# Chthi/Ofighters

Measured on AMD Instinct MI355X. Metric: arena-steps/sec (env.step+obs+policy fwd) at 4096 arenas, 1/2/4/8 MI355X, higher is better.
Workload: dtype f32; 1 GPU; 4096 arenas x 8 ships per GPU, random-bot actions + step + 2D obs rasterise (u8 maps) + bi-head policy forward for 8 ship(s)/arena, trunk shared per arena (BASELINE configs[3]); arenas_per_gpu=4096, ships=8, laser_cap=512, episode_ticks=200, parallelism=arena-sharded x1, RCCL all-reduce of episodic scores only, laser_overflow=0, last_episode_score_sum=70993, last_episode_arenas=4096

## Files before the change

### include/ofx.h

```cpp
#ifndef OFX_H
#define OFX_H

#include <stddef.h>
#include <stdint.h>

#ifdef __cplusplus
extern "C" {
#endif

#define OFX_VERSION 1

enum {
  OFX_OK = 0,
  OFX_ERR_INVALID = -1,
  OFX_ERR_NO_DEVICE = -2,
  OFX_ERR_HIP = -3,
  OFX_ERR_STATE = -4,
  OFX_ERR_OVERFLOW = -5
};

typedef struct ofx_config {
  int32_t n_arenas;
  int32_t n_ships;
  int32_t laser_cap;
// ... 102 lines not shown
int ofx_field_desc(ofx_handle *h, int field, ofx_tensor_desc *out);
int ofx_map_desc(ofx_handle *h, int map_type, int which, ofx_tensor_desc *out);

int ofx_overflow_count(ofx_handle *h, int64_t *count_host);

int ofx_episode_scores(ofx_handle *h, int64_t *sums);
int ofx_scores_allreduce(ofx_handle *h, void *nccl_comm, int64_t *sums);

int ofx_scratch_feed(ofx_handle *h, const int32_t *layers_host, int32_t n_layers,
                     const double *weights, const double *biases, const double *x,
                     int32_t batch, double *y, int32_t *argmax);
int ofx_scratch_feed_obs(ofx_handle *h, const int32_t *layers_host, int32_t n_layers,
                         const double *weights, const double *biases, double *y,
                         int32_t *argmax);

typedef struct ofx_policy_desc {
  int32_t n_floats;
  int32_t offset[64];
  int32_t count[64];
  int32_t n_tensors;
} ofx_policy_desc;
int ofx_policy_layout(const ofx_handle *h, ofx_policy_desc *desc_host);
int ofx_policy_forward(ofx_handle *h, const float *weights, const uint8_t *ship_mask,
                       float *act_values, int32_t *iaction, int32_t *ipointer,
                       float *heatmap);
int ofx_policy_pin_weights(ofx_handle *h, const float *weights);
#define OFX_OPT_TRUNK_PLAIN 1
#define OFX_OPT_FRAMES_REF  2
#define OFX_OPT_TRUNK_FUSE  4
#define OFX_OPT_BILINEAR_LEGACY 3
#define OFX_OPT_POLICY_BF16 5
#define OFX_OPT_FIT_PLAIN 6
#define OFX_OPT_TRUNK_SPARSE 7
int ofx_policy_trunk_stats(ofx_handle *h, int64_t *counts_host);
int ofx_set_option(ofx_handle *h, int32_t option, int32_t value);
int ofx_policy_explore(ofx_handle *h, double epsilon, uint64_t seed, uint32_t tick, int32_t collecting,
                       const uint8_t *ship_mask, int32_t *iaction, int32_t *ipointer);
int ofx_policy_actions(ofx_handle *h, const int32_t *iaction, const int32_t *ipointer,
                       const uint8_t *ship_mask, ofx_action *actions);

typedef struct ofx_transition {
  int32_t tick_prev, tick_next;
  int32_t frame_prev, frame_next;
  int32_t ship;
  int32_t iaction, px, py;
  int32_t reward;
  int32_t done;
  float head_prev[8], head_next[8];
} ofx_transition;
int ofx_replay_create(ofx_handle *h, int32_t capacity, int32_t frames);
int ofx_replay_destroy(ofx_handle *h);
int ofx_replay_capture(ofx_handle *h, uint32_t tick, const uint8_t *ship_mask, const int32_t *iaction,
                       const int32_t *ipointer);
int ofx_agents_first_done(ofx_handle *h, const uint8_t *ship_mask, uint8_t *seen, int32_t *count_host);
int ofx_replay_count(ofx_handle *h, int32_t *count_host, int64_t *appended_host);
int ofx_replay_rows_host(ofx_handle *h, int32_t arena, ofx_transition *rows_host, int32_t *n_host);
int ofx_replay_frame_host(ofx_handle *h, int32_t arena, int32_t tick, void *ship_bits_host, void *laser_bits_host);
int ofx_replay_sample(ofx_handle *h, uint64_t seed, uint32_t draw, int32_t batch, int32_t *slot, int32_t *n_sampled);
int ofx_replay_gather(ofx_handle *h, const int32_t *slot, int32_t batch, ofx_transition *rows, void *bits_prev,
                      void *bits_next);
int ofx_replay_gather_valid(ofx_handle *h, const int32_t *slot, const int32_t *n_sampled, int32_t batch, int32_t first,
                            int32_t max_rows, ofx_transition *rows, void *bits_prev, void *bits_next,
                            int32_t *n_rows_host);

int ofx_replay_prioritize(ofx_handle *h, float alpha, float eps);
int ofx_replay_sample_prioritized(ofx_handle *h, uint64_t seed, uint32_t draw, int32_t batch, double beta, int32_t *slot,
// ... 41 lines not shown
```

### ofighters_amd/_native.py

```python
import ctypes as C
import os

_HERE = os.path.dirname(os.path.abspath(__file__))
LIB_PATH = os.path.join(_HERE, "libofx.so")

OFX_OK = 0
OFX_ERR_INVALID = -1
OFX_ERR_NO_DEVICE = -2
OFX_ERR_HIP = -3
OFX_ERR_STATE = -4
OFX_ERR_OVERFLOW = -5

BOT_IDLE, BOT_RANDOM, BOT_TURRET, BOT_RUNNER, BOT_THRUST, BOT_SHOOT = range(6)
BEHAVIOURS = {None: BOT_IDLE, "idle": BOT_IDLE, "random": BOT_RANDOM, "turret": BOT_TURRET,
              "runner": BOT_RUNNER, "thrust": BOT_THRUST, "shoot": BOT_SHOOT}

(F_SHIP_X, F_SHIP_Y, F_SHIP_PX, F_SHIP_PY, F_SHIP_ALIVE, F_REWARD, F_SCORE, F_N_LASERS, F_LASER_X, F_LASER_Y,
 F_LASER_OWNER, F_LASER_DEAD, F_KILLER, F_TIME, F_LAST_SCORES, F_HULL, F_LASER_DX, F_LASER_DY,
 F_OBS_REWARD) = range(19)

MAP_U8, MAP_F32, MAP_F64, MAP_BITS = range(4)
OPT_TRUNK_PLAIN, OPT_FRAMES_REF, OPT_BILINEAR_LEGACY, OPT_TRUNK_FUSE, OPT_POLICY_BF16, OPT_FIT_PLAIN, OPT_TRUNK_SPARSE = 1, 2, 3, 4, 5, 6, 7


class OfxError(Exception):
    def __init__(self, code, msg):
        super().__init__(msg)
        self.code = code


class OfxConfig(C.Structure):
    _fields_ = [(n, C.c_int32) for n in (
        "n_arenas", "n_ships", "laser_cap", "width", "height", "ship_radius", "laser_radius",
        "ship_speed", "laser_speed", "reward_death", "reward_kill", "reward_aim",
        "reward_trajectory", "episode_ticks", "device", "arena_base")]


class OfxAction(C.Structure):
    _fields_ = [("px", C.c_int32), ("py", C.c_int32), ("shoot", C.c_uint8), ("thrust", C.c_uint8),
                ("valid", C.c_uint8), ("_pad", C.c_uint8)]


class OfxTransition(C.Structure):
    _fields_ = [("tick_prev", C.c_int32), ("tick_next", C.c_int32), ("frame_prev", C.c_int32),
                ("frame_next", C.c_int32), ("ship", C.c_int32), ("iaction", C.c_int32),
                ("px", C.c_int32), ("py", C.c_int32), ("reward", C.c_int32), ("done", C.c_int32),
                ("head_prev", C.c_float * 8), ("head_next", C.c_float * 8)]


class OfxTensorDesc(C.Structure):
    _fields_ = [("data", C.c_void_p), ("dtype", C.c_int32), ("itemsize", C.c_int32), ("ndim", C.c_int32),
                ("device", C.c_int32), ("shape", C.c_int64 * 4), ("stride", C.c_int64 * 4)]


DT_U8, DT_I16, DT_I32, DT_I64, DT_F32, DT_F64 = range(6)
# ... 114 lines not shown
```

### ofighters_amd/csrc/ofx_head.h

```cpp
#pragma once
#include "ofx_internal.h"

struct HeadParams2 {
  int S;
  const float *up1;
  const float *w2mf, *b2;
  const float *w2raw;
  const float *w3mf, *b3;
  const float *w3raw;
  const float *w4eff_c, *b4;
  const float *w4raw;
  const float *w2fr, *w3fr;
  const float *efr;
  float *u2fr;
  float *vfr;
  float *c4;
  const uint8_t *mask;
  int32_t *live;
  int live_ready;
  unsigned long long *best;
  float *heat;
  const int32_t *probe;
  float *ptr_probe;
  int frames_ref;
  int legacy;
  int bf16;
  int event_base;
  int ablate;
  unsigned long long *dbg;
};

size_t ofx_head_frame_bytes(size_t S, size_t *u2fr, size_t *vfr, size_t *c4);
int ofx_head_compact(ofx_handle *h, int S, const uint8_t *mask, int32_t *live);
int ofx_launch_head(ofx_handle *h, const HeadParams2 &p);
```

### ofighters_amd/csrc/ofx_head.hip

```cpp
#include "ofx_head.h"
#include "ofx_lowp.h"
#include "ofx_diag.h"
#include <stdlib.h>


typedef float f32x4 __attribute__((ext_vector_type(4)));
typedef float f32x2 __attribute__((ext_vector_type(2)));
#define HD_PS 400
constexpr int HC4_ZERO = 800;
constexpr int HC4_COL = 816, HC4_CPITCH = 416;
constexpr int HC4_STRIDE = HC4_COL + 2 * HC4_CPITCH + 16;
__device__ __forceinline__ int hc4_at(int ln, int t) { return ln < 2 ? ln * 400 + t : HC4_COL + (ln - 2) * HC4_CPITCH + t; }
__device__ __forceinline__ int hc4_pad(int k) { return k < 16 ? HC4_ZERO + k : k < 32 ? HC4_COL + 400 + k - 16 : HC4_COL + HC4_CPITCH + 400 + k - 32; }

__device__ __forceinline__ void hc4_zero_block(const HeadParams2 &p, int tid, int threads) {
  if (blockIdx.x == 0)
    for (int e = tid; e < HC4_STRIDE; e += threads) p.c4[(size_t)p.S * HC4_STRIDE + e] = 0.f;
}

__device__ __forceinline__ float hd_max_raw(float x, float floor) {
  float pinf;
  asm("s_mov_b32 %0, 0x7f800000" : "=s"(pinf));
  return __builtin_amdgcn_fmed3f(x, floor, pinf);
}
// ... 205 lines not shown
}

constexpr int HG_THREADS = 256;
constexpr int HG_L1 = 0;
constexpr int HG_U3 = 0;
constexpr int HG_RB = 6400;
constexpr int HG_CB = HG_RB + 4 * 102 * 4;
constexpr int HG_TOTAL = HG_CB + 4 * 102 * 4;
static_assert(2 * 52 * 52 <= 6400, "l1p fits under u3l");

template <int CIN, int COUT, class G>
__device__ __forceinline__ float hg_corner(G get, int n, int yc, int xc, const float *w, float bias, int co, int legacy) {
  float acc = bias;
  for (int dy = 0; dy < 3; dy++) {
    const int uy = yc + dy - 1;
    if (uy < 0 || uy >= 2 * n) continue;
    int ya, yb; float wy;
    hf_taps(uy, n, ya, yb, wy, legacy);
    for (int dx = 0; dx < 3; dx++) {
      const int ux = xc + dx - 1;
      if (ux < 0 || ux >= 2 * n) continue;
      int xa, xb; float wx;
      hf_taps(ux, n, xa, xb, wx, legacy);
      for (int ci = 0; ci < CIN; ci++) {
        const float a = get(ya, xa, ci), b = get(ya, xb, ci), d = get(yb, xa, ci), g = get(yb, xb, ci);
        const float top = a + (b - a) * wx, bot = d + (g - d) * wx;
        acc += w[((dy * 3 + dx) * CIN + ci) * COUT + co] * (top + (bot - top) * wy);
      }
    }
  }
  return fmaxf(acc, 0.f);
}

__global__ __launch_bounds__(HG_THREADS) void k_head_frames(HeadParams2 p) {
  __shared__ __align__(16) float sm[HG_TOTAL];
  __shared__ float efr_s[192], w4s[72];
  const int s = hd_ship(p, (int)((blockIdx.x & ~7u) | ((blockIdx.x + (blockIdx.x >> 3)) & 7u)));
  const int tid = threadIdx.x, lane = tid & 63;
  hc4_zero_block(p, tid, HG_THREADS);
  if (s < 0) return;
  const int wv = __builtin_amdgcn_readfirstlane(tid >> 6);
  const int n16 = lane & 15, kq = lane >> 4;
  float *l1p = sm + HG_L1, *u2rb = sm + HG_RB, *u2cb = sm + HG_CB, *u3l = sm + HG_U3;

  {
    constexpr int NB = 6 * 52 + 46 * 6, NE = 2 * NB, PER = (NE + HG_THREADS - 1) / HG_THREADS;
    float v[PER];
    int at[PER];
#pragma unroll
    for (int u = 0; u < PER; u++) {
      const int e = min(u * HG_THREADS + tid, NE - 1);
      const int ci = e / NB, k = e - ci * NB;
      int r, c;
      if (k < 6 * 52) { const int rr = k / 52; r = rr < 3 ? rr : rr + 46; c = k - rr * 52; }
      else { const int k2 = k - 6 * 52, cc = k2 % 6; r = 3 + k2 / 6; c = cc < 3 ? cc : cc + 46; }
      at[u] = (ci * 52 + r) * 52 + c;
      v[u] = p.up1[(size_t)s * 5000 + (ci * 50 + min(max(r - 1, 0), 49)) * 50 + min(max(c - 1, 0), 49)];
    }
#pragma unroll
    for (int u = 0; u < PER; u++)
      if (u * HG_THREADS + tid < NE) l1p[at[u]] = v[u];
  }
  if (tid < 192) efr_s[tid] = p.efr[tid];
  if (tid < 72) w4s[tid] = p.w4raw[tid];
  __syncthreads();

  float bw2[5];
#pragma unroll
  for (int jj = 0; jj < 5; jj++) bw2[jj] = p.w2fr[(wv * 20 + 4 * jj + kq) * 16 + n16];
  float bw3[9];
#pragma unroll
  for (int jj = 0; jj < 9; jj++) bw3[jj] = p.w3fr[(wv * 36 + 4 * jj + kq) * 16 + n16];
#pragma unroll 1
  for (int m = 0; m < 4; m++) {
    const int v = wv;
    const int pp = min(16 * m + n16, 49);
    const int i = v == 0 ? 0 : v == 1 ? 49 : pp, j = v == 2 ? 0 : v == 3 ? 49 : pp;
    const float bias = p.b2[n16 & 3];
    f32x4 d = {bias, bias, bias, bias};
#pragma unroll
    for (int jj = 0; jj < 5; jj++) {
      const int tap = min(2 * jj + (kq >> 1), 8);
      const float a = l1p[((kq & 1) * 52 + i + tap / 3) * 52 + j + tap % 3];
      d = __builtin_amdgcn_mfma_f32_16x16x4f32(a, bw2[jj], d, 0, 0, 0);
    }
    const int co = n16 & 3, pa = n16 >> 3, pb = (n16 >> 2) & 1;
#pragma unroll
    for (int r = 0; r < 4; r++) {
      const int q = 16 * m + 4 * kq + r;
      if (q >= 50) continue;
      const float val = fmaxf(d[r], 0.f);
      if (v < 2) {
        u2rb[((2 * v + pa) * 102 + 2 * q + pb + 1) * 4 + co] = val;
      } else {
        u2cb[((2 * (v - 2) + pb) * 102 + 2 * q + pa + 1) * 4 + co] = val;
      }
    }
  }
  __syncthreads();
  if (tid < 64) {
    const int co = tid & 3, cx = (tid >> 2) & 1, cy = (tid >> 3) & 1, bx = (tid >> 4) & 1, by = tid >> 5;
    const int y = by ? 98 + cy : cy, x = bx ? 98 + cx : cx;
    const int rb = by ? 2 + cy : cy, cb = bx ? 2 + cx : cx;
    const bool fy = y == 0 || y == 99, fx = x == 0 || x == 99;
    float val;
    if (fy && fx) {
      auto get = [&](int yy, int xx, int ci) { return l1p[(ci * 52 + yy + 1) * 52 + xx + 1]; };
      val = hg_corner<2, 4>(get, 50, y, x, p.w2raw, p.b2[co], co, p.legacy);
    } else if (fx) {
      val = u2cb[(cb * 102 + y + 1) * 4 + co];
    } else {
      val = u2rb[(rb * 102 + x + 1) * 4 + co];
    }
    if (fy && fx) { u2rb[(rb * 102 + x + 1) * 4 + co] = val; u2cb[(cb * 102 + y + 1) * 4 + co] = val; }
    else if (fx) u2rb[(rb * 102 + x + 1) * 4 + co] = val;
    else u2cb[(cb * 102 + y + 1) * 4 + co] = val;
  }
  __syncthreads();
  if (tid < 128) {
    const int co = tid & 3, b = (tid >> 2) & 3, hi = (tid >> 4) & 1, isc = tid >> 5;
    if (isc < 2) {
      float *ln = (isc ? u2cb : u2rb) + b * 102 * 4;
      ln[(hi ? 101 : 0) * 4 + co] = ln[(hi ? 100 : 1) * 4 + co];
    }
  }
  for (int e = tid; e < 4 * 100 * 4; e += HG_THREADS) {
    const int ln = e / 400, r = e - ln * 400;
    const float *src = ln < 2 ? u2rb + (ln ? 3 : 0) * 408 : u2cb + (ln == 3 ? 3 : 0) * 408;
    p.u2fr[(size_t)s * 1600 + e] = src[4 + r];
  }
  __syncthreads();

#pragma unroll 1
  for (int m = 0; m < 7; m++) {
    const int v = wv;
    const int qq = min(16 * m + n16, 99);
    const float *band = (v < 2 ? u2rb : u2cb);
    const int b0 = (v & 1) ? 2 : 0;
    const float bias = p.b3[n16 & 7];
    f32x4 d = {bias, bias, bias, bias};
#pragma unroll
    for (int jj = 0; jj < 9; jj++) {
      const int ty = jj / 3, tx = jj % 3;
      const int tf = v < 2 ? ty : tx, ta = v < 2 ? tx : ty;
      const int bsel = (v & 1) ? b0 + min(tf, 1) : b0 + max(tf - 1, 0);
      const float a = band[(bsel * 102 + qq + ta) * 4 + kq];
      d = __builtin_amdgcn_mfma_f32_16x16x4f32(a, bw3[jj], d, 0, 0, 0);
    }
    const int co = n16 & 7, par = n16 >> 3;
#pragma unroll
    for (int r = 0; r < 4; r++) {
      const int q = 16 * m + 4 * kq + r;
      if (q < 100) u3l[(v * 200 + 2 * q + par) * 8 + co] = fmaxf(d[r], 0.f);
    }
  }
  __syncthreads();
  if (tid < 32) {
    const int co = tid & 7, c = tid >> 3;
    const int y = (c & 1) ? 199 : 0, x = (c & 2) ? 199 : 0;
    auto get = [&](int yy, int xx, int ci) {
      return u2rb[((yy < 50 ? yy : yy - 96) * 102 + xx + 1) * 4 + ci];
    };
    const float val = hg_corner<4, 8>(get, 100, y, x, p.w3raw, p.b3[co], co, p.legacy);
    u3l[(((c & 1) ? 1 : 0) * 200 + x) * 8 + co] = val;
    u3l[(((c & 2) ? 3 : 2) * 200 + y) * 8 + co] = val;
  }
  __syncthreads();
  if (tid < 252) {
    const int tp = tid % 9, c0 = tid / 9;
    float wt[8];
#pragma unroll
    for (int ci = 0; ci < 8; ci++) wt[ci] = w4s[tp * 8 + ci];
    float *dst = p.vfr + (size_t)s * 7200 + tid;
    for (int cell = c0; cell < 4 * 200; cell += 28) {
      const f32x4 ua = *reinterpret_cast<const f32x4 *>(u3l + cell * 8), ub = *reinterpret_cast<const f32x4 *>(u3l + cell * 8 + 4);
      float acc = 0.f;
#pragma unroll
      for (int ci = 0; ci < 4; ci++) acc = fmaf(wt[ci], ua[ci], acc);
#pragma unroll
      for (int ci = 0; ci < 4; ci++) acc = fmaf(wt[4 + ci], ub[ci], acc);
      dst[(cell - c0) * 9] = acc;
    }
  }

  for (int e = tid; e < 4 * 400; e += HG_THREADS) {
    const int ln = e / 400, t = e - ln * 400, isc = ln >> 1, side = ln & 1, jq = t >> 1, b = t & 1;
    float acc = 0.f;
    if (!isc || (t > 0 && t < 399)) {
      const float *E = efr_s + ((isc * 2 + side) * 2 + b) * 24;
      const float *L = u3l + ln * 1600;
#pragma unroll
      for (int o = 0; o < 3; o++) {
        const float *Lp = L + min(max(jq + o - 1, 0), 199) * 8;
#pragma unroll
        for (int ci = 0; ci < 8; ci++) acc += E[o * 8 + ci] * Lp[ci];
      }
      if (!isc && (t == 0 || t == 399)) {
        const int cs = t ? 1 : 0;
        const int yq = side ? 199 : 0, a = side ? 1 : 0;
        const float *E2 = efr_s + ((2 + cs) * 2 + a) * 24;
        const float *L2 = u3l + (2 + cs) * 1600;
        for (int o = 0; o < 3; o++) {
          const float *Lp = L2 + min(max(yq + o - 1, 0), 199) * 8;
          for (int ci = 0; ci < 8; ci++) acc += E2[o * 8 + ci] * Lp[ci];
        }
        const int tap = (side ? 2 : 0) * 3 + (cs ? 2 : 0);
        const float *Lc = L + (t ? 199 : 0) * 8;
        for (int ci = 0; ci < 8; ci++) acc -= p.w4raw[tap * 8 + ci] * Lc[ci];
      }
    }
    p.c4[(size_t)s * HC4_STRIDE + hc4_at(ln, t)] = acc;
  }
  if (tid < 64) p.c4[(size_t)s * HC4_STRIDE + hc4_pad(tid)] = 0.f;
}

constexpr int HS_GPR = 13;
constexpr int HS_NTILES = 325;
constexpr int HS_NS = 42;
constexpr int HS_NR3 = 16, HS_P3 = 106;
constexpr int HS_PL3 = HS_NR3 * HS_P3 + 4;
constexpr int HS_NV = 9;
constexpr int HS_NR2 = 16, HS_P2 = 56;
constexpr int HS_PL2 = (HS_NR2 + 2) * HS_P2;
static_assert(HS_PL2 % 32 == 16, "uprelu2 plane stride");
constexpr int HS_TABP = 16 * HS_GPR;
static_assert(HS_TABP == 4 * 52, "table period in tiles");
static_assert(4 * (HS_NV * HS_PL3 + 4 * HS_PL2 + HS_TABP + 400) <= 80 * 1024, "two workgroups per CU");
struct alignas(16) HsPick { signed char v[HS_NS][4]; };
constexpr int hs_pairs_done_c(int s) { return s + 2 + ((s + 2) >> 2) < 50 ? s + 2 + ((s + 2) >> 2) : 50; }
constexpr HsPick hs_make_pick() {
  HsPick t{};
  for (int st = 0; st < HS_NS; st++)
    for (int cw = 0; cw < 4; cw++) {
      const int lo = 2 * hs_pairs_done_c(st), hi = 2 * hs_pairs_done_c(st + 1);
      const int at = lo + ((cw - lo) & 3);
      t.v[st][cw] = (signed char)(at < hi ? at >> 1 : -1);
    }
  return t;
}
__constant__ HsPick kHsPick = hs_make_pick();

__device__ __forceinline__ int hs_tiles_done(int s) {
  return s < 0 ? 0 : min(HS_NTILES, 8 * (s + 1) + ((s + 1) >> 3));
}

typedef const volatile __attribute__((address_space(3))) f32x2 hs_lds_v2;
// ... 486 lines not shown

int ofx_head_compact(ofx_handle *h, int S, const uint8_t *mask, int32_t *live) {
  hipLaunchKernelGGL(k_head_compact, dim3(1), dim3(1024), 0, h->stream, S, mask, live);
  OFX_HIP(hipGetLastError());
  return OFX_OK;
}

size_t ofx_head_frame_bytes(size_t S, size_t *u2fr, size_t *vfr, size_t *c4) {
  *u2fr = 4 * S * 1600;
  *vfr = 4 * S * 7200;
  *c4 = 4 * (S + 1) * HC4_STRIDE;
  return *u2fr + *vfr + *c4;
}

int ofx_launch_head(ofx_handle *h, const HeadParams2 &p0) {
  HeadParams2 p = p0;
#if OFX_HEAD_HOOKS
  { const char *e = getenv("OFX_HEAD_ABLATE"); p.ablate = e ? atoi(e) : 0; }
  static unsigned long long *dbg = nullptr;
  static int dbg_calls = 0;
  const unsigned dbg_blocks = (unsigned)(((p.S + 7) / 8) * 16);
  p.dbg = nullptr;
  if (getenv("OFX_HEAD_STAMPS")) {
    if (!dbg) (void)hipMalloc(&dbg, (size_t)dbg_blocks * 6 * (HS_NB + 4) * 8);
    if (++dbg_calls == 20) p.dbg = dbg;
  }
#endif
  if (p.mask) {
    if (!p.live) { ofx_set_error("ofx_launch_head: a mask needs the live-list scratch"); return OFX_ERR_STATE; }
    if (!p.live_ready) hipLaunchKernelGGL(k_head_compact, dim3(1), dim3(1024), 0, h->stream, p.S, p.mask, p.live);
  } else {
    p.live = nullptr;
  }
  if (p.frames_ref) hipLaunchKernelGGL(k_head_frames_ref, dim3((unsigned)p.S), dim3(HF_THREADS), 0, h->stream, p);
  else hipLaunchKernelGGL(k_head_frames, dim3((unsigned)((p.S + 7) & ~7)), dim3(HG_THREADS), 0, h->stream, p);
  OFX_HIP(hipGetLastError());
  const unsigned blocks = (unsigned)(((p.S + 7) / 8) * 16);
  int rc;
  if (p.event_base >= 0 && (rc = ofx_event_record(h, p.event_base))) return rc;
  const bool extra = p.heat || p.ptr_probe;
#define HS_LAUNCH(E, L) hipLaunchKernelGGL((k_head_stream<E, L>), dim3(blocks), dim3(HS_THREADS), 0, h->stream, p)
  if (p.bf16 == 1) { if (extra) HS_LAUNCH(true, 1); else HS_LAUNCH(false, 1); }
  else if (p.bf16 == 2) { if (extra) HS_LAUNCH(true, 2); else HS_LAUNCH(false, 2); }
  else { if (extra) HS_LAUNCH(true, 0); else HS_LAUNCH(false, 0); }
#undef HS_LAUNCH
  OFX_HIP(hipGetLastError());
  if (p.event_base >= 0 && (rc = ofx_event_record(h, p.event_base + 1))) return rc;
#if OFX_HEAD_HOOKS
  if (p.dbg) {
    (void)hipStreamSynchronize(h->stream);
    unsigned long long *hst = (unsigned long long *)malloc((size_t)blocks * 6 * (HS_NB + 4) * 8);
    (void)hipMemcpy(hst, p.dbg, (size_t)blocks * 6 * (HS_NB + 4) * 8, hipMemcpyDeviceToHost);
    double sum[2][6] = {{0}};
    for (unsigned b = 0; b < blocks; b++)
      for (int w = 0; w < HS_NB + 4; w++)
        for (int i = 0; i < 6; i++) sum[w >= HS_NB][i] += (double)hst[((size_t)b * (HS_NB + 4) + w) * 6 + i] / (w >= HS_NB ? 4.0 : (double)HS_NB);
    for (int r = 0; r < 2; r++) {
      fprintf(stderr, "head stamps %s (cycles per wave and sub-step):", r ? "C" : "B");
      for (int i = 0; i < 6; i++) fprintf(stderr, " %.0f", sum[r][i] / ((double)blocks * HS_NS));
      fprintf(stderr, "\n");
    }
    free(hst);
  }
#endif
  return OFX_OK;
}
```

### ofighters_amd/csrc/ofx_internal.h

```cpp
#pragma once
#include <hip/hip_runtime.h>
#include <stdint.h>
#include <stdio.h>

#include "../../include/ofx.h"

#define OFX_WAVE 64
#define OFX_ARENAS_PER_BLOCK 4

void ofx_set_error(const char *fmt, ...);

#define OFX_HIP(call)                                                                  \
  do {                                                                                 \
    hipError_t _e = (call);                                                            \
    if (_e != hipSuccess) {                                                            \
      ofx_set_error("%s failed: %s (%s:%d)", #call, hipGetErrorString(_e), __FILE__,   \
                    __LINE__);                                                         \
      return OFX_ERR_HIP;                                                              \
    }                                                                                  \
  } while (0)

struct ofx_state {
  int32_t *ship_x, *ship_y, *ship_px, *ship_py, *hull;
  int32_t *reward, *score, *obs_reward, *last_score;
// ... 12 lines not shown
  ofx_config cfg;
  hipStream_t stream;
  bool own_stream;
  bool spawned;
  ofx_state st;
  double hit_thresh;
  void *maps[5][2];
  int32_t *bot_behaviours;
  void *scratch;
  size_t scratch_bytes;
  hipEvent_t ev0, ev1;
  bool events;
  hipEvent_t *ring;
  int ring_n;
  int prof_base;
  ofx_replay *replay;
  void *aux;
  size_t aux_bytes;
  void *fitws;
  size_t fitws_bytes;
  void *fitws2;
  size_t fitws2_bytes;
  int32_t *counter;
  float *prep;
  float *prep_tmp;
  const float *prep_pinned;
  int opt_trunk_fuse;
  int n_cus;
  bool opt_trunk_plain, opt_frames_ref, opt_bilinear_legacy;
  int opt_policy_lowp;
  bool opt_fit_plain;
  bool opt_trunk_sparse;
  unsigned long long *trunk_stat;
};
#define OFX_RING_MAX 65536

int ofx_launch_step(ofx_handle *h, const ofx_action *actions);
int ofx_launch_raster(ofx_handle *h, int map_type, void *ship_map, void *laser_map);
int ofx_ensure_scratch(ofx_handle *h, size_t bytes);
void ofx_replay_free(ofx_handle *h);
int ofx_replay_episode_reset(ofx_handle *h, const uint8_t *arena_mask);
int ofx_launch_gemm(ofx_handle *h, const float *A, int lda, const float *B, int ldb, const float *bias, float *C, int ldc,
                    int M, int N, int K, int relu, const int32_t *live = nullptr);
int ofx_launch_conv1_lut(ofx_handle *h, const void *bits, int n, const float *lut, float *out);
int ofx_policy_weights_updated(ofx_handle *h, const float *weights);
int ofx_policy_predict_obs(ofx_handle *h, const float *weights, int32_t n_obs, const void *bits, const float *vec8,
                           float *act_values, float *heatmap, float *ptr_max);

#define OFX_MAP_BITS_LSB 4

__host__ __device__ inline void ofx_philox4x32_10(uint32_t c0, uint32_t c1, uint32_t c2, uint32_t c3,
                                                  uint32_t k0, uint32_t k1, uint32_t out[4]) {
#pragma unroll
  for (int r = 0; r < 10; r++) {
    uint64_t p0 = (uint64_t)0xD2511F53u * c0, p1 = (uint64_t)0xCD9E8D57u * c2;
    uint32_t n0 = (uint32_t)(p1 >> 32) ^ c1 ^ k0, n1 = (uint32_t)p1;
    uint32_t n2 = (uint32_t)(p0 >> 32) ^ c3 ^ k1, n3 = (uint32_t)p0;
    c0 = n0; c1 = n1; c2 = n2; c3 = n3;
    k0 += 0x9E3779B9u;
    k1 += 0xBB67AE85u;
  }
  out[0] = c0; out[1] = c1; out[2] = c2; out[3] = c3;
}
#define OFX_STREAM_BOT 0u
#define OFX_STREAM_RESET 1u

// ... 4 lines not shown
```

### ofighters_amd/csrc/ofx_policy.hip

```cpp
#include <stdlib.h>
#include <string.h>
#include <type_traits>
#include <utility>

#include "ofx_internal.h"
#include "ofx_head.h"
#include "ofx_diag.h"
#include "ofx_lowp.h"

#define PS 400

typedef float f32x4 __attribute__((ext_vector_type(4)));
typedef float f32x2 __attribute__((ext_vector_type(2)));
typedef float f32x16 __attribute__((ext_vector_type(16)));

static const int kTrunkCin[4] = {2, 8, 8, 8};
static const int kUpCin[4] = {1, 2, 4, 8};
static const int kUpCout[4] = {2, 4, 8, 1};

static int policy_layout(int32_t *offset, int32_t *count) {
  int n = 0, off = 0;
#define T(c) do { offset[n] = off; count[n] = (c); off += (c); n++; } while (0)
  for (int i = 0; i < 4; i++) { T(9 * kTrunkCin[i] * 8); T(8); T(8); T(8); T(8); T(8); }
  T(5008 * 100); T(100);
// ... 1451 lines not shown

int ofx_policy_weights_updated(ofx_handle *h, const float *weights) {
  if (h->prep_pinned && h->prep_pinned == weights) return policy_prepare(h, weights, &h->prep);
  return OFX_OK;
}

extern "C" int ofx_policy_trunk_stats(ofx_handle *h, int64_t *counts_host) {
  if (!h || !counts_host) { ofx_set_error("ofx_policy_trunk_stats: null argument"); return OFX_ERR_INVALID; }
  for (int i = 0; i < 4; i++) counts_host[i] = 0;
  if (!h->trunk_stat) return OFX_OK;
  OFX_HIP(hipSetDevice(h->cfg.device));
  OFX_HIP(hipMemcpyAsync(counts_host, h->trunk_stat, 4 * sizeof(unsigned long long), hipMemcpyDeviceToHost, h->stream));
  OFX_HIP(hipMemsetAsync(h->trunk_stat, 0, 4 * sizeof(unsigned long long), h->stream));
  OFX_HIP(hipStreamSynchronize(h->stream));
  return OFX_OK;
}

extern "C" int ofx_set_option(ofx_handle *h, int32_t option, int32_t value) {
  if (!h) { ofx_set_error("ofx_set_option: null handle"); return OFX_ERR_INVALID; }
  switch (option) {
    case OFX_OPT_TRUNK_PLAIN: h->opt_trunk_plain = value != 0; return OFX_OK;
    case OFX_OPT_TRUNK_FUSE:
      if (value < 0 || value > 2) { ofx_set_error("ofx_set_option: OFX_OPT_TRUNK_FUSE takes 0 (auto), 1 (always), 2 (never)"); return OFX_ERR_INVALID; }
      h->opt_trunk_fuse = value; return OFX_OK;
    case OFX_OPT_FRAMES_REF: h->opt_frames_ref = value != 0; return OFX_OK;
    case OFX_OPT_TRUNK_SPARSE:
      if (value && !h->trunk_stat) {
        OFX_HIP(hipSetDevice(h->cfg.device));
        OFX_HIP(hipMalloc((void **)&h->trunk_stat, 4 * sizeof(unsigned long long)));
        OFX_HIP(hipMemsetAsync(h->trunk_stat, 0, 4 * sizeof(unsigned long long), h->stream));
      }
      h->opt_trunk_sparse = value != 0; return OFX_OK;
    case OFX_OPT_FIT_PLAIN: h->opt_fit_plain = value != 0; return OFX_OK;
    case OFX_OPT_POLICY_BF16:
      if (value < 0 || value > 2) { ofx_set_error("ofx_set_option: OFX_OPT_POLICY_BF16 takes 0 (fp32), 1 (bf16 operands), 2 (fp16 operands)"); return OFX_ERR_INVALID; }
      h->opt_policy_lowp = value; return OFX_OK;
    case OFX_OPT_BILINEAR_LEGACY:
      if (h->opt_bilinear_legacy == (value != 0)) return OFX_OK;
      h->opt_bilinear_legacy = value != 0;
      OFX_HIP(hipSetDevice(h->cfg.device));
      return h->prep_pinned ? policy_prepare(h, h->prep_pinned, &h->prep) : OFX_OK;
    default: ofx_set_error("ofx_set_option: unknown option %d", option); return OFX_ERR_INVALID;
  }
}

static int policy_forward_impl(ofx_handle *h, const float *weights, int N, int M, const unsigned *bits0,
                               const unsigned *bits1, size_t bits_stride, const float *vec8, const uint8_t *ship_mask,
                               float *act_values, int32_t *iaction, int32_t *ipointer, float *heatmap, float *ptr_max,
                               const int32_t *probe, float *ptr_probe) {
  const int S = N * M;
  PolicyWs ws;
  int rc = policy_workspace(h, &ws, N, S);
  if (rc) return rc;
  int32_t off[64], cnt[64];
  policy_layout(off, cnt);
  const PrepLayout L = prep_layout();

  const bool pinned = h->prep && h->prep_pinned == weights;
  if (!pinned && (rc = policy_prepare(h, weights, &h->prep_tmp))) return rc;
  const float *prep = pinned ? h->prep : h->prep_tmp;

  ConvParams cp;
  memset(&cp, 0, sizeof(cp));
  cp.bits[0] = bits0;
  cp.bits[1] = bits1;
  cp.bits_stride = bits_stride;
// ... 39 lines not shown
  if (plain) rc = launch_conv<8, 8, 10, 50, 0, true, true>(h, cp, N, 50);
  else if (lowp == 1 && fused12) rc = launch_convm<8, 10, 4, 0, true, 1, 1>(h, cp, N, 50);
  else if (lowp == 2 && fused12) rc = launch_convm<8, 10, 4, 0, true, 1, 2>(h, cp, N, 50);
  else rc = launch_convm<8, 10, 4, 0, true, 1>(h, cp, N, 50);
  if (rc) return rc;

  const float *k1 = weights + off[t_d1];
  {
    const int tiles = ((N + 31) / 32) * 4, jobs = tiles * kDense1Chunks;
    hipLaunchKernelGGL(k_gemm_f32_splitk, dim3((jobs + 3) / 4), dim3(256), 0, h->stream, ws.p4, 5000, k1 + 8 * 100, 100,
                       ws.g1, N, 100, 5000 / kDense1Chunks, tiles, jobs);
    OFX_HIP(hipGetLastError());
  }
  HeadParams hp;
  hp.N = N; hp.M = M; hp.st = h->st; hp.vec8 = vec8; hp.g1 = ws.g1; hp.g1_chunks = kDense1Chunks;
  hp.k1 = k1; hp.b1 = weights + off[t_d1 + 1];
  hp.k2 = weights + off[t_d2]; hp.b2 = weights + off[t_d2 + 1];
  hp.k3 = weights + off[t_o1]; hp.b3 = weights + off[t_o1 + 1];
  const int32_t *live = nullptr;
  if (ship_mask) {
    if ((rc = ofx_head_compact(h, S, ship_mask, ws.live))) return rc;
    live = ws.live;
  }
  hp.mask = ship_mask; hp.live = live; hp.d1 = ws.d1; hp.act = act_values; hp.iaction = iaction ? iaction : ws.iaction;
  hipLaunchKernelGGL(k_head_dense, dim3((S + 3) / 4), dim3(256), 0, h->stream, hp);
  OFX_HIP(hipGetLastError());

  if ((rc = ofx_launch_gemm(h, ws.d1, 100, weights + off[t_ud], 625, weights + off[t_ud + 1], ws.u0, 625, S, 625, 100, 1, live)))
    return rc;
  ConvParams up;
  memset(&up, 0, sizeof(up));
  up.live = live; up.images = S; up.legacy = h->opt_bilinear_legacy;
  up.in = ws.u0; up.w = prep + L.uw[0]; up.b = prep + L.ub[0]; up.out = ws.up1;
  hipLaunchKernelGGL(k_upconv1, dim3((unsigned)(live && S > 4096 ? 4096 : S)), dim3(256), 0, h->stream, up);
  OFX_HIP(hipGetLastError());
  OFX_HIP(hipMemsetAsync(ws.best, 0, sizeof(unsigned long long) * S, h->stream));
  HeadParams2 hp2;
  memset(&hp2, 0, sizeof(hp2));
  hp2.S = S; hp2.up1 = ws.up1;
  hp2.w2mf = prep + L.w2mf; hp2.b2 = prep + L.ub[1]; hp2.w2raw = prep + L.uw[1];
  hp2.w3mf = prep + L.w3mf; hp2.b3 = prep + L.ub[2]; hp2.w3raw = prep + L.uw[2];
  hp2.w4eff_c = prep + L.w4eff_c; hp2.b4 = prep + L.b4; hp2.w4raw = prep + L.w4raw;
  hp2.w2fr = prep + L.w2fr; hp2.w3fr = prep + L.w3fr; hp2.efr = prep + L.efr;
  hp2.u2fr = ws.u2fr; hp2.vfr = ws.vfr; hp2.c4 = ws.c4;
  hp2.frames_ref = h->opt_frames_ref; hp2.legacy = h->opt_bilinear_legacy;
  hp2.bf16 = lowp;
  hp2.mask = ship_mask; hp2.live = ws.live; hp2.live_ready = ship_mask != nullptr; hp2.best = ws.best; hp2.heat = heatmap; hp2.probe = probe; hp2.ptr_probe = probe ? ptr_probe : nullptr;
  const int pb = h->prof_base;
  hp2.event_base = pb;
  if ((rc = ofx_launch_head(h, hp2))) return rc;
  if (pb >= 0) h->prof_base = pb + 3 < OFX_RING_MAX ? pb + 2 : -1;
  hipLaunchKernelGGL(k_policy_finish, dim3((S + 255) / 256), dim3(256), 0, h->stream, S, ship_mask, ws.best,
                     ipointer ? ipointer : ws.ipointer, ptr_max);
  OFX_HIP(hipGetLastError());
  return OFX_OK;
}

extern "C" int ofx_policy_forward(ofx_handle *h, const float *weights, const uint8_t *ship_mask, float *act_values,
                                  int32_t *iaction, int32_t *ipointer, float *heatmap) {
  if (!h || !weights) { ofx_set_error("ofx_policy_forward: null argument"); return OFX_ERR_INVALID; }
  if (!h->spawned) { ofx_set_error("You must execute analyse_battleground first."); return OFX_ERR_STATE; }
  const ofx_config &c = h->cfg;
  if (c.width != PS || c.height != PS) {
    ofx_set_error("ofx_policy_forward: the pointer_model takes 400x400 maps (got %d x %d)", c.width, c.height);
    return OFX_ERR_INVALID;
  }
  OFX_HIP(hipSetDevice(c.device));
  int rc = ofx_launch_raster(h, OFX_MAP_BITS_LSB, nullptr, nullptr);
  if (rc) return rc;
  return policy_forward_impl(h, weights, c.n_arenas, c.n_ships, (const unsigned *)h->maps[OFX_MAP_BITS_LSB][0],
                             (const unsigned *)h->maps[OFX_MAP_BITS_LSB][1], (size_t)(PS * PS) >> 5, nullptr, ship_mask,
                             act_values, iaction, ipointer, heatmap, nullptr, nullptr, nullptr);
// ... 161 lines not shown
```

Baseline: 220,500 arena-steps/s.

## Fuse first upconv stage into head-frames kernel as default path

Adds k_head_front, which loads each ship's 25x25 u0 plane into shared memory, upsamples bilinearly, applies the first 3x3 conv plus ReLU, and writes both the global up1 buffer and the padded frame into shared memory. It then runs the rest of the head-frames work in the same kernel, now factored out as hg_tail. This drops the separate k_upconv1 launch and the global round-trip of up1 before the head-frames kernel. The fused kernel becomes the default unless frames_ref is set or the option is 2. The u2fr and c4 store loops are also unrolled per lane. The fused kernel loops over ships with a capped grid and uses more shared memory, which may lower occupancy compared with the separate kernels.

After: 221,800 arena-steps/s (median of 6 runs). Within noise of the previous version (+0.6%).

```diff
diff --git a/include/ofx.h b/include/ofx.h
--- a/include/ofx.h
+++ b/include/ofx.h
@@ -158,6 +158,7 @@
 #define OFX_OPT_POLICY_BF16 5
 #define OFX_OPT_FIT_PLAIN 6
 #define OFX_OPT_TRUNK_SPARSE 7
+#define OFX_OPT_HEAD_FRONT 8
 int ofx_policy_trunk_stats(ofx_handle *h, int64_t *counts_host);
 int ofx_set_option(ofx_handle *h, int32_t option, int32_t value);
 int ofx_policy_explore(ofx_handle *h, double epsilon, uint64_t seed, uint32_t tick, int32_t collecting,
diff --git a/ofighters_amd/_native.py b/ofighters_amd/_native.py
--- a/ofighters_amd/_native.py
+++ b/ofighters_amd/_native.py
@@ -20,7 +20,7 @@
  F_OBS_REWARD) = range(19)
 
 MAP_U8, MAP_F32, MAP_F64, MAP_BITS = range(4)
-OPT_TRUNK_PLAIN, OPT_FRAMES_REF, OPT_BILINEAR_LEGACY, OPT_TRUNK_FUSE, OPT_POLICY_BF16, OPT_FIT_PLAIN, OPT_TRUNK_SPARSE = 1, 2, 3, 4, 5, 6, 7
+OPT_TRUNK_PLAIN, OPT_FRAMES_REF, OPT_BILINEAR_LEGACY, OPT_TRUNK_FUSE, OPT_POLICY_BF16, OPT_FIT_PLAIN, OPT_TRUNK_SPARSE, OPT_HEAD_FRONT = 1, 2, 3, 4, 5, 6, 7, 8
 
 
 class OfxError(Exception):
diff --git a/ofighters_amd/csrc/ofx_head.h b/ofighters_amd/csrc/ofx_head.h
--- a/ofighters_amd/csrc/ofx_head.h
+++ b/ofighters_amd/csrc/ofx_head.h
@@ -3,7 +3,7 @@
 
 struct HeadParams2 {
   int S;
-  const float *up1;
+  float *up1;
   const float *w2mf, *b2;
   const float *w2raw;
   const float *w3mf, *b3;
@@ -28,6 +28,8 @@
   int event_base;
   int ablate;
   unsigned long long *dbg;
+  const float *u0, *w1, *b1;
+  int front;
 };
 
 size_t ofx_head_frame_bytes(size_t S, size_t *u2fr, size_t *vfr, size_t *c4);
diff --git a/ofighters_amd/csrc/ofx_head.hip b/ofighters_amd/csrc/ofx_head.hip
--- a/ofighters_amd/csrc/ofx_head.hip
+++ b/ofighters_amd/csrc/ofx_head.hip
@@ -261,39 +261,11 @@
   return fmaxf(acc, 0.f);
 }
 
-__global__ __launch_bounds__(HG_THREADS) void k_head_frames(HeadParams2 p) {
-  __shared__ __align__(16) float sm[HG_TOTAL];
-  __shared__ float efr_s[192], w4s[72];
-  const int s = hd_ship(p, (int)((blockIdx.x & ~7u) | ((blockIdx.x + (blockIdx.x >> 3)) & 7u)));
-  const int tid = threadIdx.x, lane = tid & 63;
-  hc4_zero_block(p, tid, HG_THREADS);
-  if (s < 0) return;
+__device__ __forceinline__ void hg_tail(const HeadParams2 &p, const int s, const int tid, float *sm, const float *efr_s, const float *w4s) {
+  const int lane = tid & 63;
   const int wv = __builtin_amdgcn_readfirstlane(tid >> 6);
   const int n16 = lane & 15, kq = lane >> 4;
   float *l1p = sm + HG_L1, *u2rb = sm + HG_RB, *u2cb = sm + HG_CB, *u3l = sm + HG_U3;
-
-  {
-    constexpr int NB = 6 * 52 + 46 * 6, NE = 2 * NB, PER = (NE + HG_THREADS - 1) / HG_THREADS;
-    float v[PER];
-    int at[PER];
-#pragma unroll
-    for (int u = 0; u < PER; u++) {
-      const int e = min(u * HG_THREADS + tid, NE - 1);
-      const int ci = e / NB, k = e - ci * NB;
-      int r, c;
-      if (k < 6 * 52) { const int rr = k / 52; r = rr < 3 ? rr : rr + 46; c = k - rr * 52; }
-      else { const int k2 = k - 6 * 52, cc = k2 % 6; r = 3 + k2 / 6; c = cc < 3 ? cc : cc + 46; }
-      at[u] = (ci * 52 + r) * 52 + c;
-      v[u] = p.up1[(size_t)s * 5000 + (ci * 50 + min(max(r - 1, 0), 49)) * 50 + min(max(c - 1, 0), 49)];
-    }
-#pragma unroll
-    for (int u = 0; u < PER; u++)
-      if (u * HG_THREADS + tid < NE) l1p[at[u]] = v[u];
-  }
-  if (tid < 192) efr_s[tid] = p.efr[tid];
-  if (tid < 72) w4s[tid] = p.w4raw[tid];
-  __syncthreads();
-
   float bw2[5];
 #pragma unroll
   for (int jj = 0; jj < 5; jj++) bw2[jj] = p.w2fr[(wv * 20 + 4 * jj + kq) * 16 + n16];
@@ -353,10 +325,12 @@
       ln[(hi ? 101 : 0) * 4 + co] = ln[(hi ? 100 : 1) * 4 + co];
     }
   }
-  for (int e = tid; e < 4 * 100 * 4; e += HG_THREADS) {
-    const int ln = e / 400, r = e - ln * 400;
+#pragma unroll
+  for (int ln = 0; ln < 4; ln++) {
     const float *src = ln < 2 ? u2rb + (ln ? 3 : 0) * 408 : u2cb + (ln == 3 ? 3 : 0) * 408;
-    p.u2fr[(size_t)s * 1600 + e] = src[4 + r];
+    float *dst = p.u2fr + (size_t)s * 1600 + ln * 400;
+    dst[tid] = src[4 + tid];
+    if (tid < 400 - HG_THREADS) dst[HG_THREADS + tid] = src[4 + HG_THREADS + tid];
   }
   __syncthreads();
 
@@ -412,8 +386,8 @@
     }
   }
 
-  for (int e = tid; e < 4 * 400; e += HG_THREADS) {
-    const int ln = e / 400, t = e - ln * 400, isc = ln >> 1, side = ln & 1, jq = t >> 1, b = t & 1;
+  auto c4_pixel = [&](const int ln, const int t) {
+    const int isc = ln >> 1, side = ln & 1, jq = t >> 1, b = t & 1;
     float acc = 0.f;
     if (!isc || (t > 0 && t < 399)) {
       const float *E = efr_s + ((isc * 2 + side) * 2 + b) * 24;
@@ -439,8 +413,143 @@
       }
     }
     p.c4[(size_t)s * HC4_STRIDE + hc4_at(ln, t)] = acc;
+  };
+#pragma unroll
+  for (int ln = 0; ln < 4; ln++) {
+    c4_pixel(ln, tid);
+    if (tid < 400 - HG_THREADS) c4_pixel(ln, HG_THREADS + tid);
   }
   if (tid < 64) p.c4[(size_t)s * HC4_STRIDE + hc4_pad(tid)] = 0.f;
+}
+
+__global__ __launch_bounds__(HG_THREADS) void k_head_frames(HeadParams2 p) {
+  __shared__ __align__(16) float sm[HG_TOTAL];
+  __shared__ float efr_s[192], w4s[72];
+  const int s = hd_ship(p, (int)((blockIdx.x & ~7u) | ((blockIdx.x + (blockIdx.x >> 3)) & 7u)));
+  const int tid = threadIdx.x;
+  hc4_zero_block(p, tid, HG_THREADS);
+  if (s < 0) return;
+  float *l1p = sm + HG_L1;
+
+  {
+    constexpr int NB = 6 * 52 + 46 * 6, NE = 2 * NB, PER = (NE + HG_THREADS - 1) / HG_THREADS;
+    float v[PER];
+    int at[PER];
+#pragma unroll
+    for (int u = 0; u < PER; u++) {
+      const int e = min(u * HG_THREADS + tid, NE - 1);
+      const int ci = e / NB, k = e - ci * NB;
+      int r, c;
+      if (k < 6 * 52) { const int rr = k / 52; r = rr < 3 ? rr : rr + 46; c = k - rr * 52; }
+      else { const int k2 = k - 6 * 52, cc = k2 % 6; r = 3 + k2 / 6; c = cc < 3 ? cc : cc + 46; }
+      at[u] = (ci * 52 + r) * 52 + c;
+      v[u] = p.up1[(size_t)s * 5000 + (ci * 50 + min(max(r - 1, 0), 49)) * 50 + min(max(c - 1, 0), 49)];
+    }
+#pragma unroll
+    for (int u = 0; u < PER; u++)
+      if (u * HG_THREADS + tid < NE) l1p[at[u]] = v[u];
+  }
+  if (tid < 192) efr_s[tid] = p.efr[tid];
+  if (tid < 72) w4s[tid] = p.w4raw[tid];
+  __syncthreads();
+
+  hg_tail(p, s, tid, sm, efr_s, w4s);
+}
+
+constexpr int HG_UP = 2 * 52 * 52;
+constexpr int HG_U0 = HG_UP + 52 * 53;
+static_assert(HG_U0 + 625 <= HG_TOTAL, "the up-sampled plane and u0 fit behind l1p");
+
+template <bool LEGACY>
+__device__ __forceinline__ void hg_upsample(const float *u0s, float *up, int tid) {
+  constexpr float wE = LEGACY ? 0.f : 0.75f, wO = LEGACY ? 0.5f : 0.25f;
+  constexpr int e0 = LEGACY ? 1 : 0;
+  for (int e = tid; e < 625; e += HG_THREADS) {
+    const int ky = e / 25, kx = e - 25 * ky;
+    const int yy[3] = {max(ky - 1, 0), ky, min(ky + 1, 24)}, xx[3] = {max(kx - 1, 0), kx, min(kx + 1, 24)};
+    float he[3], ho[3];
+#pragma unroll
+    for (int r = LEGACY ? 1 : 0; r < 3; r++) {
+      const float L[3] = {u0s[yy[r] * 25 + xx[0]], u0s[yy[r] * 25 + xx[1]], u0s[yy[r] * 25 + xx[2]]};
+      he[r] = L[e0] + (L[e0 + 1] - L[e0]) * wE;
+      ho[r] = L[1] + (L[2] - L[1]) * wO;
+    }
+    float *o = up + (2 * ky + 1) * 53 + 2 * kx + 1;
+    o[0] = he[e0] + (he[e0 + 1] - he[e0]) * wE;
+    o[1] = ho[e0] + (ho[e0 + 1] - ho[e0]) * wE;
+    o[53] = he[1] + (he[2] - he[1]) * wO;
+    o[54] = ho[1] + (ho[2] - ho[1]) * wO;
+  }
+}
+
+__global__ __launch_bounds__(HG_THREADS) void k_head_front(HeadParams2 p) {
+  __shared__ __align__(16) float sm[HG_TOTAL];
+  __shared__ float efr_s[192], w4s[72];
+  __shared__ int zero_s;
+  hc4_zero_block(p, threadIdx.x, HG_THREADS);
+  if (threadIdx.x < 192) efr_s[threadIdx.x] = p.efr[threadIdx.x];
+  if (threadIdx.x < 72) w4s[threadIdx.x] = p.w4raw[threadIdx.x];
+  if (threadIdx.x == 0) zero_s = 0;
+  float *l1p = sm + HG_L1, *up = sm + HG_UP, *u0s = sm + HG_U0;
+  const int n_items = p.live ? p.live[0] : p.S, n_pad = (n_items + 7) & ~7;
+#pragma unroll 1
+  for (int it = blockIdx.x; it < n_pad; it += gridDim.x) {
+    const int s = hd_ship(p, (it & ~7) | ((it + (it >> 3)) & 7));
+    if (s < 0) continue;
+    __syncthreads();
+    const int tid = threadIdx.x + *(volatile int *)&zero_s;
+    for (int e = tid; e < 625; e += HG_THREADS) u0s[e] = p.u0[(size_t)s * 625 + e];
+    if (tid < 52) { up[tid] = 0.f; up[51 * 53 + tid] = 0.f; up[tid * 53] = 0.f; up[tid * 53 + 51] = 0.f; }
+    __syncthreads();
+    if (p.legacy) hg_upsample<true>(u0s, up, tid); else hg_upsample<false>(u0s, up, tid);
+    __syncthreads();
+    if (tid < 250) {
+      const int row = tid / 5, x0 = 10 * (tid - 5 * row);
+      float acc[2][10];
+#pragma unroll
+      for (int co = 0; co < 2; co++)
+#pragma unroll
+        for (int i = 0; i < 10; i++) acc[co][i] = 0.f;
+#pragma unroll
+      for (int dy = 0; dy < 3; dy++) {
+        float v[12];
+#pragma unroll
+        for (int i = 0; i < 12; i++) v[i] = up[(row + dy) * 53 + x0 + i];
+#pragma unroll
+        for (int dx = 0; dx < 3; dx++)
+#pragma unroll
+          for (int co = 0; co < 2; co++) {
+            const float wv = p.w1[(dy * 3 + dx) * 2 + co];
+#pragma unroll
+            for (int i = 0; i < 10; i++) acc[co][i] = __builtin_fmaf(v[i + dx], wv, acc[co][i]);
+          }
+      }
+      const int dr = row == 0 ? -52 : row == 49 ? 52 : 0;
+      const bool frame_row = row < 2 || row >= 48;
+#pragma unroll
+      for (int co = 0; co < 2; co++) {
+        const float bias = p.b1[co];
+        float *o = p.up1 + (((size_t)s * 2 + co) * 50 + row) * 50 + x0;
+        float *q = l1p + (co * 52 + row + 1) * 52 + x0 + 1;
+#pragma unroll
+        for (int i = 0; i < 10; i++) acc[co][i] = fmaxf(acc[co][i] + bias, 0.f);
+#pragma unroll
+        for (int i = 0; i < 10; i += 2) *reinterpret_cast<float2 *>(o + i) = make_float2(acc[co][i], acc[co][i + 1]);
+#pragma unroll
+        for (int i = 0; i < 10; i++) {
+          const bool lo = i < 2 && x0 == 0, hi = i >= 8 && x0 == 40;
+          if (!(frame_row || lo || hi)) continue;
+          const float val = acc[co][i];
+          q[i] = val;
+          if (dr) q[i + dr] = val;
+          const int dc = (i == 0 && lo) ? -1 : (i == 9 && hi) ? 1 : 0;
+          if (dc) { q[i + dc] = val; if (dr) q[i + dr + dc] = val; }
+        }
+      }
+    }
+    __syncthreads();
+    hg_tail(p, s, tid, sm, efr_s, w4s);
+  }
 }
 
 constexpr int HS_GPR = 13;
@@ -993,7 +1102,10 @@
   } else {
     p.live = nullptr;
   }
-  if (p.frames_ref) hipLaunchKernelGGL(k_head_frames_ref, dim3((unsigned)p.S), dim3(HF_THREADS), 0, h->stream, p);
+  if (p.front) {
+    const unsigned g = (unsigned)((p.S + 7) & ~7);
+    hipLaunchKernelGGL(k_head_front, dim3(p.live && g > 4096 ? 4096 : g), dim3(HG_THREADS), 0, h->stream, p);
+  } else if (p.frames_ref) hipLaunchKernelGGL(k_head_frames_ref, dim3((unsigned)p.S), dim3(HF_THREADS), 0, h->stream, p);
   else hipLaunchKernelGGL(k_head_frames, dim3((unsigned)((p.S + 7) & ~7)), dim3(HG_THREADS), 0, h->stream, p);
   OFX_HIP(hipGetLastError());
   const unsigned blocks = (unsigned)(((p.S + 7) / 8) * 16);
diff --git a/ofighters_amd/csrc/ofx_internal.h b/ofighters_amd/csrc/ofx_internal.h
--- a/ofighters_amd/csrc/ofx_internal.h
+++ b/ofighters_amd/csrc/ofx_internal.h
@@ -68,6 +68,7 @@
   bool opt_fit_plain;
   bool opt_trunk_sparse;
   unsigned long long *trunk_stat;
+  int opt_head_front;
 };
 #define OFX_RING_MAX 65536
 
diff --git a/ofighters_amd/csrc/ofx_policy.hip b/ofighters_amd/csrc/ofx_policy.hip
--- a/ofighters_amd/csrc/ofx_policy.hip
+++ b/ofighters_amd/csrc/ofx_policy.hip
@@ -1507,6 +1507,9 @@
       }
       h->opt_trunk_sparse = value != 0; return OFX_OK;
     case OFX_OPT_FIT_PLAIN: h->opt_fit_plain = value != 0; return OFX_OK;
+    case OFX_OPT_HEAD_FRONT:
+      if (value != 0 && value != 2) { ofx_set_error("ofx_set_option: OFX_OPT_HEAD_FRONT takes 0 (the library's choice: fused) or 2 (k_upconv1 + k_head_frames)"); return OFX_ERR_INVALID; }
+      h->opt_head_front = value; return OFX_OK;
     case OFX_OPT_POLICY_BF16:
       if (value < 0 || value > 2) { ofx_set_error("ofx_set_option: OFX_OPT_POLICY_BF16 takes 0 (fp32), 1 (bf16 operands), 2 (fp16 operands)"); return OFX_ERR_INVALID; }
       h->opt_policy_lowp = value; return OFX_OK;
@@ -1612,12 +1615,16 @@
   memset(&up, 0, sizeof(up));
   up.live = live; up.images = S; up.legacy = h->opt_bilinear_legacy;
   up.in = ws.u0; up.w = prep + L.uw[0]; up.b = prep + L.ub[0]; up.out = ws.up1;
-  hipLaunchKernelGGL(k_upconv1, dim3((unsigned)(live && S > 4096 ? 4096 : S)), dim3(256), 0, h->stream, up);
-  OFX_HIP(hipGetLastError());
+  const bool front = h->opt_head_front != 2 && !h->opt_frames_ref;
+  if (!front) {
+    hipLaunchKernelGGL(k_upconv1, dim3((unsigned)(live && S > 4096 ? 4096 : S)), dim3(256), 0, h->stream, up);
+    OFX_HIP(hipGetLastError());
+  }
   OFX_HIP(hipMemsetAsync(ws.best, 0, sizeof(unsigned long long) * S, h->stream));
   HeadParams2 hp2;
   memset(&hp2, 0, sizeof(hp2));
   hp2.S = S; hp2.up1 = ws.up1;
+  hp2.front = front; hp2.u0 = ws.u0; hp2.w1 = up.w; hp2.b1 = up.b;
   hp2.w2mf = prep + L.w2mf; hp2.b2 = prep + L.ub[1]; hp2.w2raw = prep + L.uw[1];
   hp2.w3mf = prep + L.w3mf; hp2.b3 = prep + L.ub[2]; hp2.w3raw = prep + L.uw[2];
   hp2.w4eff_c = prep + L.w4eff_c; hp2.b4 = prep + L.b4; hp2.w4raw = prep + L.w4raw;
```
